# Tani843/Mixed_Precision_Multigrid_Solvers_for_PDEs

Measured on AMD Instinct MI355X. Metric: MDoF/s per V-cycle on 2D Poisson, higher is better.
Workload: dtype f64 (adaptive policy); 1 GPU; 2D Poisson 4097^2 adaptive fp32->fp64 (switch_threshold=1e-6), V(2,2) weighted-Jacobi omega=0.8, 11 levels, 1xMI355X; levels=11, cycle=V(2,2), smoother=jacobi, parallelism=1 GPU

## Files before the change

### include/mghip.h

```cpp
#ifndef MGHIP_H
#define MGHIP_H

#include <stdint.h>

#ifdef __cplusplus
extern "C" {
#endif

#define MG_OK 0
#define MG_ERR_INVALID_VALUE (-1)
#define MG_ERR_NO_DEVICE (-2)
#define MG_ERR_HIP (-3)
#define MG_ERR_STATE (-4)
#define MG_ERR_ALLOC (-5)

typedef enum { MG_F32 = 0, MG_F64 = 1 } mg_dtype;
typedef enum {
  MG_JACOBI = 0,
  MG_RBGS = 1,
  MG_LEXGS = 2
} mg_smoother_t;
typedef enum { MG_CYCLE_V = 0, MG_CYCLE_W = 1, MG_CYCLE_F = 2 } mg_cycle_t;
typedef enum {
  MG_PREC_DOUBLE = 0,
// ... 16 lines not shown
  double coarse_tol;
  int32_t coarse_maxit;
  int32_t precision;
  double switch_threshold;
  double memory_threshold_gb;
  int32_t adaptive_reference_rule;
  int32_t device;
  int32_t profile;
  int32_t colour_offset;
  int32_t fused;
  int32_t tail;
  int32_t fmg_cycles;
  int32_t speculate;
  int32_t coarse_direct;
  int32_t mixed_split;
} mg_config;

typedef struct mg_stats {
  double solve_seconds;
  double h2d_seconds;
  double d2h_seconds;
  double initial_residual;
  int32_t precision_switches;
  int32_t last_coarse_sweeps;
  int32_t switch_reason;
  double fp32_floor;
} mg_stats;

typedef struct mg_handle mg_handle;

// ... 145 lines not shown
```

### mixed_precision_multigrid_solvers_for_pdes_amd/_lib.py

```python
import ctypes as C
import os

import numpy as np

from . import _build

MG_OK = 0
MG_ERR_INVALID_VALUE, MG_ERR_NO_DEVICE, MG_ERR_HIP, MG_ERR_STATE, MG_ERR_ALLOC, MG_ERR_TIMEOUT = -1, -2, -3, -4, -5, -6
MG_PLAN_PHASES = 7
PLAN_PHASE_NAMES = ("legs", "halo_copy", "halo_exchange", "coarse_allgather", "replicated_engine", "allreduce", "other")


class PlanTimeout(RuntimeError):
    """mg_plan_wait gave up (MG_ERR_TIMEOUT): the queued device work is still queued, so the process must not
    synchronise on it again -- report and leave (distributed.bench_main does, with os._exit)."""
MG_F32, MG_F64 = 0, 1
MG_JACOBI, MG_RBGS, MG_LEXGS = 0, 1, 2
MG_CYCLE_V, MG_CYCLE_W, MG_CYCLE_F = 0, 1, 2
MG_PREC_DOUBLE, MG_PREC_SINGLE, MG_PREC_MIXED_LEVELS, MG_PREC_ADAPTIVE, MG_PREC_SINGLE_MANAGED, MG_PREC_DEFECT = 0, 1, 2, 3, 4, 5

CYCLES = {"V": MG_CYCLE_V, "W": MG_CYCLE_W, "F": MG_CYCLE_F}


class MgConfig(C.Structure):
    _fields_ = [
        ("nx", C.c_int32), ("ny", C.c_int32),
        ("x0", C.c_double), ("x1", C.c_double), ("y0", C.c_double), ("y1", C.c_double),
        ("coeff", C.c_double),
        ("max_levels", C.c_int32), ("cycle", C.c_int32), ("pre", C.c_int32), ("post", C.c_int32),
        ("smoother", C.c_int32),
        ("omega", C.c_double),
        ("coarse_tol", C.c_double), ("coarse_maxit", C.c_int32),
        ("precision", C.c_int32),
        ("switch_threshold", C.c_double), ("memory_threshold_gb", C.c_double),
        ("adaptive_reference_rule", C.c_int32),
        ("device", C.c_int32), ("profile", C.c_int32), ("colour_offset", C.c_int32), ("fused", C.c_int32),
        ("tail", C.c_int32), ("fmg_cycles", C.c_int32), ("speculate", C.c_int32), ("coarse_direct", C.c_int32),
        ("mixed_split", C.c_int32),
    ]


class MgStats(C.Structure):
    _fields_ = [
        ("solve_seconds", C.c_double), ("h2d_seconds", C.c_double), ("d2h_seconds", C.c_double),
        ("initial_residual", C.c_double),
        ("precision_switches", C.c_int32), ("last_coarse_sweeps", C.c_int32),
        ("switch_reason", C.c_int32), ("fp32_floor", C.c_double),
    ]


SWITCH_REASONS = {0: None, 1: "threshold", 2: "stagnation", 3: "fp32_floor", 4: "fp32_skipped"}


# ... 195 lines not shown
```

### mixed_precision_multigrid_solvers_for_pdes_amd/csrc/mg_engine.hip

```cpp
#include "mg_launch.hpp"

#include <cstring>

namespace mgh {

std::string& last_error() {
  thread_local std::string msg;
  return msg;
}

static int upload(std::string* err, void* dev, int ddt, int ld, const void* host, int hdt, int nx, int ny, void* staging,
           hipStream_t st) {
  if (ddt == hdt) {
    HIPC(err, hipMemcpy2DAsync(dev, (size_t)ld * esize(ddt), host, (size_t)ny * esize(hdt), (size_t)ny * esize(hdt), nx,
                               hipMemcpyHostToDevice, st));
  } else {
    const int lds = pitch_elems(hdt, ny);
    HIPC(err, hipMemcpy2DAsync(staging, (size_t)lds * esize(hdt), host, (size_t)ny * esize(hdt), (size_t)ny * esize(hdt),
                               nx, hipMemcpyHostToDevice, st));
    d_convert(hdt, ddt, staging, dev, nx, ny, lds, ld, st);
  }
  HIPC(err, hipStreamSynchronize(st));
  return MG_OK;
}
// ... 267 lines not shown
  if ((tail2 || tail_lds) && h->cfg.tail != 0) {
    if (h->tail_direct && h->tail_minv_sigma != h->sigma) { const int rc = build_coarse_inverse(h); if (rc != MG_OK) return rc; }
    if (tail2) return tail2_launch(h, zero_u);
    launch_tail(h, zero_u);
    return MG_OK;
  }
  if (l == L - 1) {
    coarse_solve(h, l, zero_u);
    return MG_OK;
  }
  Level& c = h->lv[l + 1];
  const int dc = h->level_dtype(l + 1);
  const bool fine = (l == 0);
  const int sm = h->cfg.smoother;
  LegGeom g = leg_geom(h, l, dt, dc);
  if (part != kPartBack) {
    StageTimer tm(h, &f, 0);
    if (h->cfg.pre > 2 && zero_u) { (void)hipMemsetAsync(f.u[dt], 0, bytes, h->stream); zero_u = false; }
    extra_sweeps(h, f, dt, g, h->cfg.pre - 2);
    g.nsweep = std::min(2, h->cfg.pre);
    d_down(sm, dt, dc, f.u[dt], f.rhs[dt], f.t[dt], c.rhs[dc], g, zero_u, h->stream);
    std::swap(f.u[dt], f.t[dt]);
  }
  for (int k = 0, n = h->visits(l); k < n && part != kPartBack; ++k) {
    const int rc = cycle_fused(h, l + 1, k == 0);
    if (rc != MG_OK) return rc;
  }
  if (part != kPartFront) {
    StageTimer tm(h, &f, 2);
    const bool want_norm = fine && h->cfg.post <= 2 && h->cfg.precision != MG_PREC_DEFECT;
    g.nsweep = std::min(2, h->cfg.post);
    const int n = d_up(sm, dt, dc, h->grid_dtype, f.u[dt], f.rhs[dt], f.t[dt], c.u[dc], h->partials, g, want_norm, h->stream);
    if (n < 0) return MG_ERR_INVALID_VALUE;
    std::swap(f.u[dt], f.t[dt]);
    if (fine) h->norm_partials = want_norm ? n : 0;
    extra_sweeps(h, f, dt, g, h->cfg.post - 2);
  }
  return MG_OK;
}

bool span_ok(const mg_handle* h) {
  if (h->cfg.speculate < 2 || !h->fused() || h->L() < 3 || h->varcoef) return false;
  if (h->cfg.pre < 1 || h->cfg.pre > 2 || h->cfg.post < 1 || h->cfg.post > 2 || h->cfg.precision == MG_PREC_DEFECT) return false;
  if (!use_rb(leg_geom(h, 0, h->level_dtype(0), h->level_dtype(1)))) return false;
  return h->level_dtype(0) == h->level_dtype(1) && (h->level_dtype(0) == MG_F32 || h->grid_dtype == MG_F64);
}
int cycle_span(mg_handle* h, bool keep_mid) {
// ... 468 lines not shown
    const int rc = run_cycle(h);
    if (rc != MG_OK) return fail(&h->err, rc, "cycle: unsupported precision combination");
  }
  HIPC(&h->err, hipGetLastError());
  return MG_OK;
}

int mg_time_op(mg_handle* h, int op, int level, int dtype, int reps, double* avg_ms) {
  if (!h || !avg_ms || reps < 1 || level < 0 || level >= h->L() || !valid_dtype(dtype))
    return fail(h ? &h->err : nullptr, MG_ERR_INVALID_VALUE, "mg_time_op: bad argument");
  HIPC(&h->err, hipSetDevice(h->cfg.device));
  Level& v = h->lv[level];
  const int dt = dtype;
  if (op != 6 && (!v.u[dt] || !v.rhs[dt])) return fail(&h->err, MG_ERR_STATE, "mg_time_op: level has no arrays of that dtype");
  if ((op == 0 || op == 10) && h->cfg.smoother != MG_JACOBI) return fail(&h->err, MG_ERR_STATE, "mg_time_op: jacobi needs a Jacobi-configured handle");
  if ((op == 0 || (op >= 7 && op <= 9)) && !v.t[dt]) return fail(&h->err, MG_ERR_STATE, "mg_time_op: no ping-pong buffer on this level");
  if ((op == 2 || op == 4 || op == 5 || op == 7 || op == 8) && (level >= h->L() - 1 || !v.r[dt])) return fail(&h->err, MG_ERR_STATE, "mg_time_op: no coarser level");
  static const int exp_nsweep = exp_env("MG_EXP_NSWEEP", 2);
  h->norm_partials = 0;
  if (level == 0 && (op == 0 || op == 1 || (op >= 5 && op <= 9) || op == 12 || op == 13)) h->iterate_zero = false;
  std::vector<void*> hbm_sets;
  struct FreeSets { std::vector<void*>& v; ~FreeSets() { for (void* p : v) (void)hipFree(p); } } free_sets{hbm_sets};
  int nsets = 0, set_idx = 0;
  if (op == 10 || op == 11) {
    const size_t bytes = (size_t)v.nx * v.ld[dt] * esize(dt);
    nsets = std::max<int>(3, (int)((768ull << 20) / (3 * bytes)) + 1);
    for (int k = 0; k < 3 * nsets; ++k) {
      void* p = nullptr;
      HIPC(&h->err, hipMalloc(&p, bytes));
      hbm_sets.push_back(p);
      HIPC(&h->err, hipMemcpyAsync(p, (k % 3 == 1) ? v.rhs[dt] : v.u[dt], bytes, hipMemcpyDeviceToDevice, h->stream));
    }
  }
  hipEvent_t e0, e1;
  HIPC(&h->err, hipEventCreate(&e0));
// ... 22 lines not shown
                  std::swap(v.u[dt], v.t[dt]); } break;
        case 8: { Level& c = h->lv[level + 1]; const int dc = c.u[dt] ? dt : 1 - dt;
                  LegGeom g = leg_geom(h, level, dt, dc); g.nsweep = exp_nsweep;
                  if (d_up(h->cfg.smoother, dt, dc, h->grid_dtype, v.u[dt], v.rhs[dt], v.t[dt], c.u[dc], h->partials, g, level == 0, h->stream) < 0) return MG_ERR_INVALID_VALUE;
                  std::swap(v.u[dt], v.t[dt]); } break;
        case 9: { LegGeom g = leg_geom(h, level, dt, -1); g.nsweep = exp_nsweep;
                  d_sweeps(h->cfg.smoother, dt, v.u[dt], v.rhs[dt], v.t[dt], g, h->stream);
                  std::swap(v.u[dt], v.t[dt]); } break;
        case 12: case 13: {
                  const int phase0 = h->phase;
                  if (h->cfg.precision == MG_PREC_ADAPTIVE) h->phase = dt;
                  const bool ok = level == 0 && span_ok(h) && h->level_dtype(0) == dt;
                  const int rc2 = ok ? cycle_span(h, op == 12) : MG_ERR_INVALID_VALUE;
                  h->phase = phase0;
                  if (rc2 != MG_OK) return rc2; } break;
        default: return MG_ERR_INVALID_VALUE;
      }
    }
    return MG_OK;
  };
  int rc = run(1);
  if (rc != MG_OK) { (void)hipEventDestroy(e0); (void)hipEventDestroy(e1); return fail(&h->err, rc, "mg_time_op: unsupported op"); }
  HIPC(&h->err, hipEventRecord(e0, h->stream));
  rc = run(reps);
  HIPC(&h->err, hipEventRecord(e1, h->stream));
  HIPC(&h->err, hipEventSynchronize(e1));
  float ms = 0;
  HIPC(&h->err, hipEventElapsedTime(&ms, e0, e1));
  (void)hipEventDestroy(e0); (void)hipEventDestroy(e1);
  *avg_ms = (double)ms / reps;
// ... 5 lines not shown
```

### mixed_precision_multigrid_solvers_for_pdes_amd/csrc/mg_kernels.hpp

```cpp
#pragma once

#include <hip/hip_runtime.h>
#include <stdint.h>
#include <type_traits>

namespace mg {

constexpr int kBlock = 256;
constexpr int kTileRowBytes = 512;
constexpr int kTI = 32;
constexpr int kNumXcd = 8;
constexpr int kCoarseTag = 0, kFineTag = 1;
constexpr int kSmJacobi = 0, kSmRbgs = 1;
__host__ __device__ constexpr int sweep_halo(int sm) { return sm == kSmRbgs ? 2 : 1; }

template <typename T> struct VecW { static constexpr int N = 16 / sizeof(T); };

template <typename T> struct alignas(16) Pack {
  T v[VecW<T>::N];
};

template <typename T> __device__ __forceinline__ Pack<T> ldg(const T* p) {
  return *reinterpret_cast<const Pack<T>*>(p);
}
// ... 1546 lines not shown
    }
  }
  Pack<T> f[S::RPT], uu[S::RPT];
#pragma unroll
  for (int k = 0; k < S::RPT; ++k) {
    const int r = r_base + k, gi = ri0 + r;
    f[k] = zero_pack<T>();
    uu[k] = zero_pack<T>();
    if (!worker || r >= S::RI) continue;
    if (gi >= 0 && gi < a.nx && gj0 >= 0 && gj0 < a.nyv && !MG_EXP_NO_LOAD) {
      f[k] = ldg(rhs + (size_t)gi * a.ld + gj0);
      if (!ZERO_INIT) uu[k] = ldg(u + (size_t)gi * a.ld + gj0);
    }
  }
  if (PROLONG) __syncthreads();
#pragma unroll
  for (int k = 0; k < S::RPT; ++k) {
    const int r = r_base + k, gi = ri0 + r;
    if (!worker || r >= S::RI) continue;
    if (PROLONG && gi >= 0 && gi < a.nx && gj0 >= 0 && gj0 < a.nyv && !MG_EXP_NO_LOAD) {
      using TS = typename std::conditional<(sizeof(TC) > sizeof(T)), TC, T>::type;
      TC val[N];
      bool ok[N];
      const TX* pe = patch - ((ptrdiff_t)pic0 * PW + pjc0);
      prolong_vec<TX, TC, N>(pe, PW, a.nxc, a.nyc, gi, gj0, a.nx, a.ny, a.sides, val, ok, a.ci_off, a.cj_off);
#pragma unroll
      for (int e = 0; e < N; ++e)
        if (ok[e]) uu[k].v[e] = (T)((TS)uu[k].v[e] + (TS)val[e]);
    }
    *reinterpret_cast<Pack<T>*>(bufA + r * S::RJ + lc) = uu[k];
  }
  __syncthreads();

  T* src = bufA;
  T* dst = bufB;
  if (SM == kSmRbgs) {
    for (int s = 0; s < 2 * a.nsweep; ++s) {
      const int colour = s & 1;
#pragma unroll
      for (int k = 0; k < S::RPT; ++k) {
        const int r = r_base + k, gi = ri0 + r;
        if (!worker || r >= S::RI) continue;
        if (r >= 1 && r < S::RI - 1 && gi >= 1 && gi < a.nx - 1) {
          const Pack<T> up = *reinterpret_cast<const Pack<T>*>(src + (r - 1) * S::RJ + lc);
          const Pack<T> mid = *reinterpret_cast<const Pack<T>*>(src + r * S::RJ + lc);
          const Pack<T> dn = *reinterpret_cast<const Pack<T>*>(src + (r + 1) * S::RJ + lc);
          const T left = src[r * S::RJ + lc - 1];
          const T right = src[r * S::RJ + lc + N];
          Pack<T> o = mid;
#pragma unroll
          for (int e = 0; e < N; ++e) {
            const T w = (e == 0) ? left : mid.v[e - 1];
// ... 6 lines not shown
              un = (f[k].v[e] + (ihx2 * sx + ihy2 * sy)) * rdv[VAR ? k : 0][VAR ? e : 0];
            } else {
              const T nb = ihx2 * (dn.v[e] + up.v[e]) + ihy2 * (ea + w);
              un = a.use_div ? (f[k].v[e] + nb) / D : (f[k].v[e] + nb) * invD;
            }
            const T res = one_m_omega * mid.v[e] + omega * un;
            const int gj = gj0 + e;
            if (gj >= 1 && gj < a.ny - 1 && (((gi + gj + a.colour_offset) & 1) == colour)) o.v[e] = res;
          }
          *reinterpret_cast<Pack<T>*>(src + r * S::RJ + lc) = o;
        }
      }
      __syncthreads();
    }
  } else
  for (int s = 0; s < (MG_EXP_NO_COMPUTE ? 0 : a.nsweep); ++s) {
    if (worker && r_base < S::RI) {
      Pack<T> up = (r_base >= 1) ? *reinterpret_cast<const Pack<T>*>(src + (r_base - 1) * S::RJ + lc) : zero_pack<T>();
      Pack<T> mid = *reinterpret_cast<const Pack<T>*>(src + r_base * S::RJ + lc);
#pragma unroll
      for (int k = 0; k < S::RPT; ++k) {
        const int r = r_base + k, gi = ri0 + r;
        if (r >= S::RI) break;
        const Pack<T> dn = (r + 1 < S::RI) ? *reinterpret_cast<const Pack<T>*>(src + (r + 1) * S::RJ + lc) : zero_pack<T>();
        Pack<T> o = mid;
        if (r >= 1 && r < S::RI - 1 && gi >= 1 && gi < a.nx - 1) {
          const T left = src[r * S::RJ + lc - 1];
          const T right = src[r * S::RJ + lc + N];
#pragma unroll
          for (int e = 0; e < N; ++e) {
            const T w = (e == 0) ? left : mid.v[e - 1];
// ... 119 lines not shown
```

### mixed_precision_multigrid_solvers_for_pdes_amd/csrc/mg_launch.hip

```cpp
#include "mg_launch.hpp"
#include "mg_rb_kernels.hpp"

#include <cstring>

namespace mgh {

int pitch_elems(int dt, int ny) {
  const size_t bytes = ((size_t)ny * esize(dt) + 511) / 512 * 512;
  return (int)(bytes / esize(dt));
}

template <typename T>
mg::TileGeom make_geom(int nx, int ny, int ld, bool interior_only) {
  using S = mg::TileShape<T>;
  mg::TileGeom g;
  g.nx = nx; g.ny = ny; g.ld = ld;
  g.nyv = std::min(ld, (ny + S::N - 1) / S::N * S::N);
  g.i_org = interior_only ? 1 : 0;
  const int rows = interior_only ? nx - 2 : nx;
  const int cols = interior_only ? ny - 1 : ny;
  const int tiles_i = (rows + mg::kTI - 1) / mg::kTI;
  g.tiles_j = (cols + S::TJ - 1) / S::TJ;
  g.ntiles = tiles_i * g.tiles_j;
  return g;
// ... 332 lines not shown
    using T = decltype(t); using TX = decltype(x); using TC = decltype(tc);
    if constexpr (!interp_ok<T, TX, TC>) return -1;
    else return with_smoother(sm, [&](auto s) {
      constexpr int SM = decltype(s)::value;
      return norm ? launch_leg_sized<kLegUpNorm, T, TX, TC, SM>(u, rhs, out, e_c, partials, g, false, st)
                  : launch_leg_sized<kLegUp, T, TX, TC, SM>(u, rhs, out, e_c, partials, g, false, st);
    });
  });
}
void d_sweeps(int sm, int dt, const void* u, const void* rhs, void* out, const LegGeom& g, hipStream_t st) {
  with_dtype(dt, [&](auto t) {
    using T = decltype(t);
    with_smoother(sm, [&](auto s) {
      launch_leg_sized<kLegSweeps, T, T, T, decltype(s)::value>(u, rhs, out, nullptr, nullptr, g, false, st);
    });
  });
}

void d_inject_ring(int di, int dout, const void* fine, void* coarse, int nxf, int nyf, int ldf, int nxc, int nyc, int ldc,
                   hipStream_t st, int sides, int ci_off, int cj_off) {
  with_dtype(di, dout, [&](auto ti, auto to) {
    using TI = decltype(ti); using TO = decltype(to);
    hipLaunchKernelGGL((mg::inject_ring_kernel<TI, TO>), dim3(grid_for(2 * (nxc + nyc))), dim3(mg::kBlock), 0, st,
                       (const TI*)fine, (TO*)coarse, nxf, nyf, ldf, nxc, nyc, ldc, sides, ci_off, cj_off);
  });
}
void d_var(int mode, int dt, const void* u, const void* a, const void* f, void* out, int nx, int ny, int ld, double hx, double hy,
           double omega, double coeff, int colour, int poff, hipStream_t st, double sigma) {
  auto go = [&](auto m) { launch_var<decltype(m)::value>(dt, u, a, f, out, nullptr, nx, ny, ld, hx, hy, omega, coeff, colour, poff, st, sigma); };
  if (mode == mg::kVarJacobi) go(std::integral_constant<int, mg::kVarJacobi>());
// ... 127 lines not shown
```

### mixed_precision_multigrid_solvers_for_pdes_amd/csrc/mg_launch.hpp

```cpp
#pragma once

#include "mg_host.hpp"

namespace mgh {

int pitch_elems(int dt, int ny);
size_t max_partials(int nx, int ny);

void d_jacobi(int dt, const void* u, const void* rhs, void* out, int nx, int ny, int ld, double hx, double hy,
              double omega, hipStream_t st, bool fine = false, double sigma = 0.0);
void d_rbgs_colour(int dt, void* u, const void* rhs, int nx, int ny, int ld, double hx, double hy, double omega,
                   int colour, int poff, hipStream_t st, bool fine = false, double sigma = 0.0);
void d_residual(int dt, const void* u, const void* f, void* r, int nx, int ny, int ld, double hx, double hy,
                double coeff, hipStream_t st, bool fine = false, double sigma = 0.0);
int d_residual_norm(int dt, const void* u, const void* f, double* partials, int nx, int ny, int ld, double hx,
                    double hy, double coeff, hipStream_t st, bool fine = false, double sigma = 0.0);
int d_sumsq(int dt, const void* x, double* partials, int ld, int i_lo, int i_hi, int j_lo, int j_hi, hipStream_t st);
void launch_reduce(const double* partials, int n, double* out, hipStream_t st, mg::HostMailbox* mailbox = nullptr,
                   unsigned long long seq = 0);
void d_restrict_sub(int di, int dout, const void* fine, void* coarse, int ldf, int nxc, int nyc, int ldc, int sides,
                    hipStream_t st);
void d_restrict(int di, int dout, const void* fine, void* coarse, int nxf, int nyf, int ldf, int ldc, hipStream_t st);
int d_prolong_sub(bool add, int dc, int df, int dcomp, const void* e, void* u, int nxf, int nyf, int ldf, int nxc, int nyc,
                  int ldc, int sides, hipStream_t st);
// ... 23 lines not shown
  int select = 0, in_i_lo = 0, in_i_hi = 0, in_j_lo = 0, in_j_hi = 0;
  double sigma = 0.0;
  const void* acoef = nullptr;
  const void* rdiag = nullptr;
  int rb = 0;
};
bool use_rb(const LegGeom& g);

int d_span(int dt, int dcomp, const void* u, const void* rhs, void* out_mid, void* out_next, const void* e_c, void* rhs_c,
           double* partials, const LegGeom& g, int nsweep_pre, hipStream_t st, int sm = MG_JACOBI);
void d_down(int sm, int dt, int dx, const void* u, const void* rhs, void* out, void* rhs_c, const LegGeom& g, bool zero_init,
            hipStream_t st);
int d_up(int sm, int dt, int dx, int dcomp, const void* u, const void* rhs, void* out, const void* e_c, double* partials,
         const LegGeom& g, bool norm, hipStream_t st);
void d_sweeps(int sm, int dt, const void* u, const void* rhs, void* out, const LegGeom& g, hipStream_t st);

constexpr size_t kTailPoolLimit = 150 * 1024;
size_t tail_pool_bytes(const mg_handle* h, int k, size_t esz, size_t esz_last);
int tail_set_attrs(size_t bytes);
void launch_tail(mg_handle* h, bool zero_top);

int launch_defect(mg_handle* h, bool update);
void d_stream_triad(int dt, const void* a, const void* b, void* out, int nx, int ny, int ld, hipStream_t st);
void d_residual_f32in_f64out(const float* u, const float* f, double* r, int nx, int ny, int ld_in, int ld_out, double hx,
                             double hy, double coeff, hipStream_t st);

}
```

### mixed_precision_multigrid_solvers_for_pdes_amd/csrc/mg_rb_kernels.hpp

```cpp
#pragma once

#include "mg_kernels.hpp"

namespace mg {

#ifndef MG_RB_HL_MIN
#define MG_RB_HL_MIN 4
#endif
template <typename T, int HALO, int W, int RPT> struct RbShape {
  static constexpr int N = VecW<T>::N;
  static constexpr int HL = (MG_RB_HL_MIN <= 2 && 2 * N >= HALO) ? 2 : ((HALO + N - 1) / N > 4 ? (HALO + N - 1) / N : 4);
  static constexpr int RI = W * RPT;
  static constexpr int RJ = 64 * N;
  static constexpr int TI = RI - 2 * HALO;
  static constexpr int TJ = (64 - 2 * HL) * N;
  static_assert(TI > 0 && TI % 2 == 0, "tile height must be even (coarse rows sit on every other tile row)");
  static_assert(RPT % 2 == 0, "rows per wave must be even (row parities are compile-time constants per strip row)");
  static_assert(HL * N >= HALO, "lateral halo too narrow");
};

#ifndef MG_RB_NT_MODE
#define MG_RB_NT_MODE 3
#endif
template <typename T> __device__ __forceinline__ T dpp_from_lower_lane(T x);
// ... 68 lines not shown
    return r;
  }
};

template <typename T, int W>
__device__ __forceinline__ void rb_exchange(Pack<T>* __restrict__ xb, int w, int lane, const Pack<T>& top, const Pack<T>& bottom,
                                            Pack<T>& above, Pack<T>& below) {
  xb[(w * 2 + 0) * 64 + lane] = top;
  xb[(w * 2 + 1) * 64 + lane] = bottom;
  __syncthreads();
  above = (w > 0) ? xb[((w - 1) * 2 + 1) * 64 + lane] : zero_pack<T>();
  below = (w < W - 1) ? xb[((w + 1) * 2 + 0) * 64 + lane] : zero_pack<T>();
}

template <typename T, int HALO, bool PROLONG, int POST, bool ZERO_INIT, typename TX, typename TC, int SM, int W, int RPT, bool INT, int NT,
          bool VAR, int SPAN = 0>
__device__ __forceinline__ void rb_leg_body(const T* __restrict__ u, const T* __restrict__ rhs, T* __restrict__ out,
                                            const TX* __restrict__ e_coarse, TX* __restrict__ rhs_coarse,
                                            double* __restrict__ partials, const FusedArgs& a, T ihx2, T ihy2, T invD, T D, T omega,
                                            T one_m_omega, T coeff, Pack<T>* __restrict__ xbuf, TX* __restrict__ patch,
                                            double* __restrict__ red, int i0, int j0, const T* __restrict__ acoef, T sigma,
                                            const T* __restrict__ rdiag, T* __restrict__ out2 = nullptr) {
  static_assert(SPAN == 0 || (PROLONG && POST == kPostRestrict && !ZERO_INIT), "a spanning leg is an up leg followed by a down leg");
  using S = RbShape<T, HALO, W, RPT>;
  constexpr int N = S::N;
  constexpr int PH = S::RI / 2 + 2, PW = S::RJ / 2 + 2;
  constexpr int kRowPar = (1 - HALO) & 1;
  const int ri0 = i0 - HALO, rj0 = j0 - S::HL * N;
  const int lane = threadIdx.x & 63, w = __builtin_amdgcn_readfirstlane(threadIdx.x >> 6);
  const int gj0 = rj0 + lane * N;
  const int r_base = w * RPT;
  const bool col_in = INT || (gj0 >= 0 && gj0 < a.nyv);

  const int pic0 = (ri0 >> 1) + a.ci_off, pjc0 = (rj0 >> 1) + a.cj_off;
  if (PROLONG) {
    for (int idx = threadIdx.x; idx < PH * PW; idx += W * 64) {
      const int pr = idx / PW, pc = idx - pr * PW;
      const int ic = pic0 + pr, jc = pjc0 + pc;
// ... 32 lines not shown
#pragma unroll
    for (int k = 0; k < RPT; ++k) {
      const Pack<T> up = (k > 0) ? A[k > 0 ? k - 1 : 0] : a_above;
      const Pack<T> dn = (k < RPT - 1) ? A[k < RPT - 1 ? k + 1 : 0] : a_below;
      const T left = dpp_from_lower_lane<T>(A[k].v[N - 1]);
      const T right = dpp_from_upper_lane<T>(A[k].v[0]);
#pragma unroll
      for (int e = 0; e < N; ++e) {
        av[VAR ? k : 0].v[e] = T(0.5) * (A[k].v[e] + up.v[e]);
        if (k == RPT - 1) av[VAR ? RPT : 0].v[e] = T(0.5) * (A[k].v[e] + dn.v[e]);
        ah[VAR ? k : 0][VAR ? e : 0] = T(0.5) * (A[k].v[e] + ((e == 0) ? left : A[k].v[e > 0 ? e - 1 : 0]));
      }
      ah[VAR ? k : 0][VAR ? N : 0] = T(0.5) * (A[k].v[N - 1] + right);
    }
  }
  if (PROLONG) {
    __syncthreads();
    using TS = typename std::conditional<(sizeof(TC) > sizeof(T)), TC, T>::type;
    if (INT) {
      constexpr int M = N / 2 + 1;
      const TX* pl = patch + (r_base / 2) * PW + lane * (N / 2);
#pragma unroll
      for (int k = 0; k < RPT; ++k) {
        const bool iodd = ((kRowPar + k) & 1) != 0;
        const int pr = (k + kRowPar) >> 1;
        TC av[M], bv[M];
#pragma unroll
        for (int m = 0; m < M; ++m) {
          av[m] = (TC)pl[pr * PW + m];
          bv[m] = iodd ? (TC)pl[(pr + 1) * PW + m] : TC(0);
        }
// ... 9 lines not shown
    } else {
      const TX* pe = patch - ((ptrdiff_t)pic0 * PW + pjc0);
#pragma unroll
      for (int k = 0; k < RPT; ++k) {
        const int gi = ri0 + r_base + k;
        if (gi >= 0 && gi < a.nx && col_in) {
          TC val[N];
          bool ok[N];
          prolong_vec<TX, TC, N>(pe, PW, a.nxc, a.nyc, gi, gj0, a.nx, a.ny, a.sides, val, ok, a.ci_off, a.cj_off);
#pragma unroll
          for (int e = 0; e < N; ++e)
            if (ok[e]) U[k].v[e] = (T)((TS)U[k].v[e] + (TS)val[e]);
        }
      }
    }
  }

  int stage = 0;
  auto run_sweeps = [&](int nsw) {
  const int npass = (SM == kSmRbgs) ? 2 * nsw : nsw;
  for (int s = 0; s < npass; ++s, ++stage) {
    Pack<T> above, below;
    rb_exchange<T, W>(xbuf + (size_t)(stage & 1) * W * 2 * 64, w, lane, U[0], U[RPT - 1], above, below);
    const int colour = s & 1;
    static_assert(N % 2 == 0 && RPT % 2 == 0, "strip rows / lane cells must be even for a workgroup-uniform colour parity");
    const int par0 = (ri0 + rj0 + a.colour_offset) & 1;
    auto pass = [&](auto qp) {
      constexpr int QP = decltype(qp)::value;
      Pack<T> prev = above;
#pragma unroll
      for (int k = 0; k < RPT; ++k) {
        const int r = r_base + k, gi = ri0 + r;
        const Pack<T> mid = U[k];
        const Pack<T> dn = (k < RPT - 1) ? U[k + 1] : below;
        const T left = dpp_from_lower_lane<T>(mid.v[N - 1]);
        const T right = dpp_from_upper_lane<T>(mid.v[0]);
// ... 20 lines not shown
            const T sx = aip * dn.v[e] + aim * prev.v[e], sy = ajp * ea + ajm * wv;
            const T un = (F[k].v[e] + (ihx2 * sx + ihy2 * sy)) * RD[VAR ? k : 0].v[e];
            const T res = one_m_omega * mid.v[e] + omega * un;
            const int gj = gj0 + e;
            if (INT || (gj >= 1 && gj < a.ny - 1)) o.v[e] = res;
          }
        }
        U[k] = o;
        prev = (SM == kSmRbgs) ? o : mid;
      }
    };
    if (SM == kSmRbgs && ((par0 + colour) & 1) != 0) pass(std::integral_constant<int, 1>{});
    else pass(std::integral_constant<int, 0>{});
  }
  };
  run_sweeps(a.nsweep);

  const bool lane_in_tile = lane >= S::HL && lane < 64 - S::HL;
  auto store_tile = [&](T* __restrict__ dst) {
#pragma unroll
    for (int k = 0; k < RPT; ++k) {
      const int r = r_base + k, gi = ri0 + r;
      if (r >= HALO && r < HALO + S::TI && lane_in_tile && (INT || (gi < a.nx && gj0 < a.nyv))) {
        if (NT & 1) stg_nt(dst + (size_t)gi * a.ld + gj0, U[k]); else stg(dst + (size_t)gi * a.ld + gj0, U[k]);
      }
    }
  };
  if (SPAN != 2) store_tile(out);
  if (POST == kPostNone) return;

  Pack<T> R[RPT];
  double acc = 0.0;
  auto residual = [&](auto norm_stage) {
    constexpr bool NORM = decltype(norm_stage)::value;
    Pack<T> above, below;
    rb_exchange<T, W>(xbuf + (size_t)(stage & 1) * W * 2 * 64, w, lane, U[0], U[RPT - 1], above, below);
    ++stage;
#pragma unroll
    for (int k = 0; k < RPT; ++k) {
      const int r = r_base + k, gi = ri0 + r;
      const Pack<T> up = (k > 0) ? U[k - 1] : above;
      const Pack<T> mid = U[k];
      const Pack<T> dn = (k < RPT - 1) ? U[k + 1] : below;
// ... 37 lines not shown
            if (NORM && in_tile && (INT || (gi >= a.ni_lo && gi < a.ni_hi && gj >= a.nj_lo && gj < a.nj_hi)))
              acc += (double)o.v[e] * (double)o.v[e];
          }
        }
      }
      R[k] = o;
    }
  };
  if (POST == kPostNorm || SPAN) {
    residual(std::true_type{});
    const double t = block_reduce_sum<W>(acc, red);
    if (threadIdx.x == 0) partials[blockIdx.x] = t;
    if (!SPAN) return;
  }
  if (SPAN) {
    run_sweeps(a.nsweep2);
    store_tile(out2);
  }
  residual(std::false_type{});

  {
    Pack<T> above, below;
    rb_exchange<T, W>(xbuf + (size_t)(stage & 1) * W * 2 * 64, w, lane, R[0], R[RPT - 1], above, below);
#pragma unroll
    for (int k = 0; k < RPT; ++k) {
      const int r = r_base + k, fi = ri0 + r;
      const Pack<T> up = (k > 0) ? R[k - 1] : above;
      const Pack<T> mid = R[k];
      const Pack<T> dn = (k < RPT - 1) ? R[k + 1] : below;
      if (((kRowPar + k) & 1) != 0) continue;
      const T nw0 = dpp_from_lower_lane<T>(up.v[N - 1]), w0 = dpp_from_lower_lane<T>(mid.v[N - 1]), sw0 = dpp_from_lower_lane<T>(dn.v[N - 1]);
// ... 3 lines not shown
#pragma unroll
      for (int e = 0; e < N; e += 2) {
        const int fj = gj0 + e, jc = (fj >> 1) + a.cj_off;
        if (!INT && (jc < 1 || jc > a.nyc - 2 || fj < 1 || fj > a.ny - 2)) continue;
        const T NWv = (e == 0) ? nw0 : up.v[e > 0 ? e - 1 : 0], Wv = (e == 0) ? w0 : mid.v[e > 0 ? e - 1 : 0],
                SWv = (e == 0) ? sw0 : dn.v[e > 0 ? e - 1 : 0];
        const T corners = ((NWv + up.v[e + 1]) + SWv) + dn.v[e + 1];
        const T edges = ((up.v[e] + dn.v[e]) + Wv) + mid.v[e + 1];
        rhs_coarse[(size_t)ic * a.ldc + jc] = (TX)((T(1.0 / 16.0) * corners + T(1.0 / 8.0) * edges) + T(1.0 / 4.0) * mid.v[e]);
      }
    }
  }
}

template <typename T, int HALO, bool PROLONG, int POST, bool ZERO_INIT, typename TX, typename TC, int TAG, int SM, int W, int RPT,
          bool VAR = false>
__global__ __launch_bounds__(W * 64, (VAR && sizeof(T) == 8) ? 4 : 1) void rb_leg_kernel(
    const T* __restrict__ u, const T* __restrict__ rhs, T* __restrict__ out,
    const TX* __restrict__ e_coarse,
    TX* __restrict__ rhs_coarse,
    double* __restrict__ partials,
    FusedArgs a, T ihx2, T ihy2, T invD, T D, T omega, T one_m_omega, T coeff,
    const T* __restrict__ acoef,
    T sigma,
    const T* __restrict__ rdiag) {
  using S = RbShape<T, HALO, W, RPT>;
  constexpr int N = S::N;
  constexpr int kNT = (TAG == 2) ? MG_RB_NT_MODE : 0;
  constexpr int PH = S::RI / 2 + 2, PW = S::RJ / 2 + 2;
  constexpr size_t kXBytes = (size_t)2 * W * 2 * 64 * sizeof(Pack<T>);
  constexpr size_t kPatchBytes = PROLONG ? (size_t)PH * PW * sizeof(TX) : 0;
// ... 12 lines not shown
    if ((a.select == 1) != inner) {
      if (POST == kPostNorm && threadIdx.x == 0) partials[blockIdx.x] = 0.0;
      return;
    }
  }
  bool interior = !(a.exp_flags & 4) && ri0 >= 1 && ri0 + S::RI <= a.nx - 1 && rj0 >= 1 && rj0 + S::RJ <= a.ny - 1;
  if (PROLONG) {
    const int pic0 = (ri0 >> 1) + a.ci_off, pjc0 = (rj0 >> 1) + a.cj_off;
    interior = interior && pic0 >= 0 && pic0 + PH <= a.nxc && pjc0 >= 0 && pjc0 + PW <= a.nyc;
  }
  if (POST == kPostNorm) interior = interior && i0 >= a.ni_lo && i0 + S::TI <= a.ni_hi && j0 >= a.nj_lo && j0 + S::TJ <= a.nj_hi;
  if (POST == kPostRestrict)
    interior = interior && ((i0 + 1) >> 1) + a.ci_off >= 1 && ((i0 + S::TI - 1) >> 1) + a.ci_off <= a.nxc - 2 &&
               (j0 >> 1) + a.cj_off >= 1 && ((j0 + S::TJ - 2) >> 1) + a.cj_off <= a.nyc - 2;
  if (interior)
    rb_leg_body<T, HALO, PROLONG, POST, ZERO_INIT, TX, TC, SM, W, RPT, true, kNT, VAR>(u, rhs, out, e_coarse, rhs_coarse, partials, a, ihx2, ihy2,
                                                                                invD, D, omega, one_m_omega, coeff, xbuf, patch, red, i0, j0,
                                                                                acoef, sigma, rdiag);
  else
    rb_leg_body<T, HALO, PROLONG, POST, ZERO_INIT, TX, TC, SM, W, RPT, false, kNT, VAR>(u, rhs, out, e_coarse, rhs_coarse, partials, a, ihx2, ihy2,
                                                                                 invD, D, omega, one_m_omega, coeff, xbuf, patch, red, i0, j0,
                                                                                 acoef, sigma, rdiag);
}

template <typename T, int HALO, typename TX, typename TC, int TAG, int SM, int W, int RPT, int SPAN>
__global__ __launch_bounds__(W * 64, 4) void rb_span_kernel(
    const T* __restrict__ u, const T* __restrict__ rhs, T* __restrict__ out_mid, T* __restrict__ out_next,
    const TX* __restrict__ e_coarse, TX* __restrict__ rhs_coarse, double* __restrict__ partials,
    FusedArgs a, T ihx2, T ihy2, T invD, T D, T omega, T one_m_omega, T coeff) {
  using S = RbShape<T, HALO, W, RPT>;
  constexpr int N = S::N;
  constexpr int kNT = (TAG == 2) ? MG_RB_NT_MODE : 0;
  constexpr int PH = S::RI / 2 + 2, PW = S::RJ / 2 + 2;
  constexpr size_t kXBytes = (size_t)2 * W * 2 * 64 * sizeof(Pack<T>);
  constexpr size_t kPatchBytes = (size_t)PH * PW * sizeof(TX);
// ... 33 lines not shown
```

### mixed_precision_multigrid_solvers_for_pdes_amd/engine.py

```python
import ctypes as C

import numpy as np

from . import _lib


def _direct_code(coarse_direct):
    import os
    if coarse_direct is None:
        coarse_direct = {"0": False, "1": True}.get(os.environ.get("MG_COARSE_DIRECT", "auto"), "auto")
    if isinstance(coarse_direct, str):
        if coarse_direct != "auto":
            raise ValueError(f"coarse_direct: True, False, 'auto' or None, not {coarse_direct!r}")
        return -1
    return int(bool(coarse_direct))


class MultigridEngine:

    def __init__(self, nx, ny, domain=(0.0, 1.0, 0.0, 1.0), coeff=-1.0, max_levels=4, cycle="V", pre=2, post=2,
                 smoother=_lib.MG_JACOBI, omega=0.8, coarse_tol=1e-12, coarse_maxit=1000,
                 precision=_lib.MG_PREC_DOUBLE, switch_threshold=1e-6, memory_threshold_gb=4.0,
                 adaptive_reference_rule=False, device=0, profile=False, colour_offset=0, fused=2, tail=True, speculate=True, fmg_cycles=0,
                 mixed_split=0, coarse_direct=None):
        lib = _lib.load()
        if isinstance(cycle, str):
            if cycle not in _lib.CYCLES:
                raise ValueError(f"unknown cycle type {cycle!r}")
            cycle = _lib.CYCLES[cycle]
        cfg = _lib.MgConfig(int(nx), int(ny), float(domain[0]), float(domain[1]), float(domain[2]), float(domain[3]),
                            float(coeff), int(max_levels), int(cycle), int(pre), int(post), int(smoother),
                            float(omega), float(coarse_tol), int(coarse_maxit), int(precision),
                            float(switch_threshold), float(memory_threshold_gb), int(bool(adaptive_reference_rule)),
                            int(device), int(bool(profile)), int(colour_offset), int(fused), int(tail), int(fmg_cycles), (2 if speculate is True else int(speculate)),
                            _direct_code(coarse_direct), int(mixed_split))
        self.cfg = cfg
        self._h = C.c_void_p(None)
        _lib.check(lib.mg_create(C.byref(cfg), C.byref(self._h)))
        self._lib = lib
        n = C.c_int(0)
        self._check(lib.mg_num_levels(self._h, C.byref(n)))
        self.num_levels = n.value
        self.shapes = []
        for l in range(self.num_levels):
            a, b = C.c_int(0), C.c_int(0)
            self._check(lib.mg_level_shape(self._h, l, C.byref(a), C.byref(b)))
            self.shapes.append((a.value, b.value))
        self.nx, self.ny = int(nx), int(ny)

    def _check(self, rc):
# ... 95 lines not shown
        self._check(self._lib.mg_fmg(self._h, int(cycles_per_level)))

    def residual_norm(self):
        out = C.c_double(0.0)
        self._check(self._lib.mg_residual_norm(self._h, C.byref(out)))
        return out.value

    def set_working_precision(self, dtype):
        self._check(self._lib.mg_set_working_precision(self._h, _lib.dtype_code(dtype)))

    def synchronize(self):
        self._check(self._lib.mg_synchronize(self._h))

    def time_op(self, op, level=0, dtype=np.float64, reps=20):
        ops = {"jacobi": 0, "rbgs": 1, "residual": 2, "residual_norm": 3, "restrict": 4, "prolong": 5, "cycle": 6,
               "down_leg": 7, "up_leg": 8, "sweeps2": 9, "jacobi_hbm": 10, "stream_hbm": 11, "span_leg": 12, "span_leg_nomid": 13}
        out = C.c_double(0.0)
        self._check(self._lib.mg_time_op(self._h, ops[op] if isinstance(op, str) else int(op), int(level),
                                         _lib.dtype_code(dtype), int(reps), C.byref(out)))
        return out.value

    def level_timings(self):
        res = {}
        for l in range(self.num_levels):
            t = (C.c_double * 3)()
            self._check(self._lib.mg_level_timings(self._h, l, t))
            res[l] = {"smooth_time": t[0], "restrict_time": t[1], "prolong_time": t[2]}
        return res
```

Before: 79320 MDoF/s.

## Recompute zero-start pre-smoothed iterate in up leg instead of storing it

On coarse levels where the iterate starts at zero, the down leg no longer writes the pre-smoothed solution. The up leg regenerates it from the rhs before adding the prolonged correction and post-smoothing. The first Jacobi sweep from a zero start is also replaced by a closed form (omega*rhs/D), which skips the neighbour exchange. This cuts HBM write and read traffic for the iterate at the cost of redoing the pre-smoothing sweeps in the up leg. A new config flag, on by default, gates the path, and timing ops are added for it.

```diff
diff --git a/include/mghip.h b/include/mghip.h
--- a/include/mghip.h
+++ b/include/mghip.h
@@ -54,6 +54,7 @@
   int32_t speculate;
   int32_t coarse_direct;
   int32_t mixed_split;
+  int32_t recompute;
 } mg_config;
 
 typedef struct mg_stats {
diff --git a/mixed_precision_multigrid_solvers_for_pdes_amd/_lib.py b/mixed_precision_multigrid_solvers_for_pdes_amd/_lib.py
--- a/mixed_precision_multigrid_solvers_for_pdes_amd/_lib.py
+++ b/mixed_precision_multigrid_solvers_for_pdes_amd/_lib.py
@@ -36,7 +36,7 @@
         ("adaptive_reference_rule", C.c_int32),
         ("device", C.c_int32), ("profile", C.c_int32), ("colour_offset", C.c_int32), ("fused", C.c_int32),
         ("tail", C.c_int32), ("fmg_cycles", C.c_int32), ("speculate", C.c_int32), ("coarse_direct", C.c_int32),
-        ("mixed_split", C.c_int32),
+        ("mixed_split", C.c_int32), ("recompute", C.c_int32),
     ]
 
 
diff --git a/mixed_precision_multigrid_solvers_for_pdes_amd/csrc/mg_engine.hip b/mixed_precision_multigrid_solvers_for_pdes_amd/csrc/mg_engine.hip
--- a/mixed_precision_multigrid_solvers_for_pdes_amd/csrc/mg_engine.hip
+++ b/mixed_precision_multigrid_solvers_for_pdes_amd/csrc/mg_engine.hip
@@ -305,13 +305,19 @@
   const bool fine = (l == 0);
   const int sm = h->cfg.smoother;
   LegGeom g = leg_geom(h, l, dt, dc);
+  const bool recompute = zero_u && l >= 1 && part == kPartFull && h->cfg.recompute != 0 && sm == MG_JACOBI && !h->varcoef &&
+                         h->cfg.pre >= 1 && h->cfg.pre <= 2 && recompute_ok(g);
   if (part != kPartBack) {
     StageTimer tm(h, &f, 0);
     if (h->cfg.pre > 2 && zero_u) { (void)hipMemsetAsync(f.u[dt], 0, bytes, h->stream); zero_u = false; }
     extra_sweeps(h, f, dt, g, h->cfg.pre - 2);
     g.nsweep = std::min(2, h->cfg.pre);
-    d_down(sm, dt, dc, f.u[dt], f.rhs[dt], f.t[dt], c.rhs[dc], g, zero_u, h->stream);
-    std::swap(f.u[dt], f.t[dt]);
+    if (recompute) {
+      d_down_nostore(dt, dc, f.rhs[dt], c.rhs[dc], g, h->stream);
+    } else {
+      d_down(sm, dt, dc, f.u[dt], f.rhs[dt], f.t[dt], c.rhs[dc], g, zero_u, h->stream);
+      std::swap(f.u[dt], f.t[dt]);
+    }
   }
   for (int k = 0, n = h->visits(l); k < n && part != kPartBack; ++k) {
     const int rc = cycle_fused(h, l + 1, k == 0);
@@ -321,7 +327,8 @@
     StageTimer tm(h, &f, 2);
     const bool want_norm = fine && h->cfg.post <= 2 && h->cfg.precision != MG_PREC_DEFECT;
     g.nsweep = std::min(2, h->cfg.post);
-    const int n = d_up(sm, dt, dc, h->grid_dtype, f.u[dt], f.rhs[dt], f.t[dt], c.u[dc], h->partials, g, want_norm, h->stream);
+    const int n = recompute ? d_up_recompute(dt, dc, h->grid_dtype, f.rhs[dt], f.t[dt], c.u[dc], g, h->cfg.pre, h->stream)
+                            : d_up(sm, dt, dc, h->grid_dtype, f.u[dt], f.rhs[dt], f.t[dt], c.u[dc], h->partials, g, want_norm, h->stream);
     if (n < 0) return MG_ERR_INVALID_VALUE;
     std::swap(f.u[dt], f.t[dt]);
     if (fine) h->norm_partials = want_norm ? n : 0;
@@ -820,11 +827,11 @@
   const int dt = dtype;
   if (op != 6 && (!v.u[dt] || !v.rhs[dt])) return fail(&h->err, MG_ERR_STATE, "mg_time_op: level has no arrays of that dtype");
   if ((op == 0 || op == 10) && h->cfg.smoother != MG_JACOBI) return fail(&h->err, MG_ERR_STATE, "mg_time_op: jacobi needs a Jacobi-configured handle");
-  if ((op == 0 || (op >= 7 && op <= 9)) && !v.t[dt]) return fail(&h->err, MG_ERR_STATE, "mg_time_op: no ping-pong buffer on this level");
-  if ((op == 2 || op == 4 || op == 5 || op == 7 || op == 8) && (level >= h->L() - 1 || !v.r[dt])) return fail(&h->err, MG_ERR_STATE, "mg_time_op: no coarser level");
+  if ((op == 0 || (op >= 7 && op <= 9) || op == 14 || op == 16) && !v.t[dt]) return fail(&h->err, MG_ERR_STATE, "mg_time_op: no ping-pong buffer on this level");
+  if ((op == 2 || op == 4 || op == 5 || op == 7 || op == 8 || (op >= 14 && op <= 16)) && (level >= h->L() - 1 || !v.r[dt])) return fail(&h->err, MG_ERR_STATE, "mg_time_op: no coarser level");
   static const int exp_nsweep = exp_env("MG_EXP_NSWEEP", 2);
   h->norm_partials = 0;
-  if (level == 0 && (op == 0 || op == 1 || (op >= 5 && op <= 9) || op == 12 || op == 13)) h->iterate_zero = false;
+  if (level == 0 && (op == 0 || op == 1 || (op >= 5 && op <= 9) || (op >= 12 && op <= 16))) h->iterate_zero = false;
   std::vector<void*> hbm_sets;
   struct FreeSets { std::vector<void*>& v; ~FreeSets() { for (void* p : v) (void)hipFree(p); } } free_sets{hbm_sets};
   int nsets = 0, set_idx = 0;
@@ -877,6 +884,18 @@
                   const int rc2 = ok ? cycle_span(h, op == 12) : MG_ERR_INVALID_VALUE;
                   h->phase = phase0;
                   if (rc2 != MG_OK) return rc2; } break;
+        case 14: case 15: case 16: {
+                  Level& c = h->lv[level + 1]; const int dc = (op == 16 ? c.u[dt] : c.rhs[dt]) ? dt : 1 - dt;
+                  LegGeom g = leg_geom(h, level, dt, dc); g.nsweep = exp_nsweep;
+                  if (op == 14) {
+                    d_down(h->cfg.smoother, dt, dc, v.u[dt], v.rhs[dt], v.t[dt], c.rhs[dc], g, true, h->stream);
+                    std::swap(v.u[dt], v.t[dt]);
+                    break;
+                  }
+                  if (h->cfg.smoother != MG_JACOBI || h->varcoef || !recompute_ok(g)) return MG_ERR_INVALID_VALUE;
+                  if (op == 15) { d_down_nostore(dt, dc, v.rhs[dt], c.rhs[dc], g, h->stream); break; }
+                  if (d_up_recompute(dt, dc, h->grid_dtype, v.rhs[dt], v.t[dt], c.u[dc], g, exp_nsweep, h->stream) < 0) return MG_ERR_INVALID_VALUE;
+                  std::swap(v.u[dt], v.t[dt]); } break;
         default: return MG_ERR_INVALID_VALUE;
       }
     }
diff --git a/mixed_precision_multigrid_solvers_for_pdes_amd/csrc/mg_kernels.hpp b/mixed_precision_multigrid_solvers_for_pdes_amd/csrc/mg_kernels.hpp
--- a/mixed_precision_multigrid_solvers_for_pdes_amd/csrc/mg_kernels.hpp
+++ b/mixed_precision_multigrid_solvers_for_pdes_amd/csrc/mg_kernels.hpp
@@ -1584,10 +1584,22 @@
     }
   }
   if (PROLONG) __syncthreads();
+  const int first_pass = (ZERO_INIT && !PROLONG && !VAR && a.nsweep >= 1 && !MG_EXP_NO_COMPUTE) ? 1 : 0;
+  const T zero_nb = ihx2 * T(0) + ihy2 * T(0);
 #pragma unroll
   for (int k = 0; k < S::RPT; ++k) {
     const int r = r_base + k, gi = ri0 + r;
     if (!worker || r >= S::RI) continue;
+    if (first_pass && gi >= 1 && gi < a.nx - 1) {
+#pragma unroll
+      for (int e = 0; e < N; ++e) {
+        const T t = f[k].v[e] + zero_nb;
+        const T un = a.use_div ? t / D : t * invD;
+        const T res = one_m_omega * T(0) + omega * un;
+        const int gj = gj0 + e;
+        if (gj >= 1 && gj < a.ny - 1 && (SM != kSmRbgs || ((gi + gj + a.colour_offset) & 1) == 0)) uu[k].v[e] = res;
+      }
+    }
     if (PROLONG && gi >= 0 && gi < a.nx && gj0 >= 0 && gj0 < a.nyv && !MG_EXP_NO_LOAD) {
       using TS = typename std::conditional<(sizeof(TC) > sizeof(T)), TC, T>::type;
       TC val[N];
@@ -1605,7 +1617,7 @@
   T* src = bufA;
   T* dst = bufB;
   if (SM == kSmRbgs) {
-    for (int s = 0; s < 2 * a.nsweep; ++s) {
+    for (int s = first_pass; s < 2 * a.nsweep; ++s) {
       const int colour = s & 1;
 #pragma unroll
       for (int k = 0; k < S::RPT; ++k) {
@@ -1642,7 +1654,7 @@
       __syncthreads();
     }
   } else
-  for (int s = 0; s < (MG_EXP_NO_COMPUTE ? 0 : a.nsweep); ++s) {
+  for (int s = first_pass; s < (MG_EXP_NO_COMPUTE ? 0 : a.nsweep); ++s) {
     if (worker && r_base < S::RI) {
       Pack<T> up = (r_base >= 1) ? *reinterpret_cast<const Pack<T>*>(src + (r_base - 1) * S::RJ + lc) : zero_pack<T>();
       Pack<T> mid = *reinterpret_cast<const Pack<T>*>(src + r_base * S::RJ + lc);
diff --git a/mixed_precision_multigrid_solvers_for_pdes_amd/csrc/mg_launch.hip b/mixed_precision_multigrid_solvers_for_pdes_amd/csrc/mg_launch.hip
--- a/mixed_precision_multigrid_solvers_for_pdes_amd/csrc/mg_launch.hip
+++ b/mixed_precision_multigrid_solvers_for_pdes_amd/csrc/mg_launch.hip
@@ -370,6 +370,38 @@
     with_smoother(sm, [&](auto s) {
       launch_leg_sized<kLegSweeps, T, T, T, decltype(s)::value>(u, rhs, out, nullptr, nullptr, g, false, st);
     });
+  });
+}
+
+bool recompute_ok(const LegGeom& g) { return use_rb(g) && !g.acoef; }
+
+template <bool UP, typename T, typename TX, typename TC>
+static void launch_recompute(const void* rhs, void* out, const void* coarse, const LegGeom& g, int nsweep_pre, hipStream_t st) {
+  constexpr int SM = mg::kSmJacobi, W = MG_EXP_RB_W, RPT = 8;
+  constexpr int HALO = 2 * mg::sweep_halo(SM) + (UP ? 1 : 2);
+  constexpr int POST = UP ? mg::kPostNone : mg::kPostRestrict;
+  const Coef c = coefs(g.hx, g.hy, g.sigma);
+  mg::FusedArgs a = rb_args<T, HALO, W, RPT>(g, !c.pow2);
+  a.nsweep2 = nsweep_pre;
+  auto k = rb_stream(g, sizeof(T)) ? mg::rb_leg_kernel<T, HALO, UP, POST, true, TX, TC, 2, SM, W, RPT, false, UP>
+                                   : mg::rb_leg_kernel<T, HALO, UP, POST, true, TX, TC, 1, SM, W, RPT, false, UP>;
+  hipLaunchKernelGGL(k, dim3(a.ntiles), dim3(W * 64), 0, st, (const T*)nullptr, (const T*)rhs, (T*)out,
+                     UP ? (const TX*)coarse : nullptr, UP ? nullptr : (TX*)coarse, (double*)nullptr, a, (T)c.ihx2, (T)c.ihy2,
+                     (T)c.invD, (T)c.diag, (T)g.omega, (T)(1.0 - g.omega), (T)(UP ? 0.0 : g.coeff), (const T*)nullptr, (T)g.sigma,
+                     (const T*)nullptr);
+}
+void d_down_nostore(int dt, int dx, const void* rhs, void* rhs_c, const LegGeom& g, hipStream_t st) {
+  with_dtype(dt, dx, [&](auto t, auto x) {
+    using T = decltype(t);
+    launch_recompute<false, T, decltype(x), T>(rhs, nullptr, rhs_c, g, 0, st);
+  });
+}
+int d_up_recompute(int dt, int dx, int dcomp, const void* rhs, void* out, const void* e_c, const LegGeom& g, int nsweep_pre,
+                   hipStream_t st) {
+  return with_dtype(dt, dx, dcomp, [&](auto t, auto x, auto tc) {
+    using T = decltype(t); using TX = decltype(x); using TC = decltype(tc);
+    if constexpr (!interp_ok<T, TX, TC>) return -1;
+    else { launch_recompute<true, T, TX, TC>(rhs, out, e_c, g, nsweep_pre, st); return 0; }
   });
 }
 
diff --git a/mixed_precision_multigrid_solvers_for_pdes_amd/csrc/mg_launch.hpp b/mixed_precision_multigrid_solvers_for_pdes_amd/csrc/mg_launch.hpp
--- a/mixed_precision_multigrid_solvers_for_pdes_amd/csrc/mg_launch.hpp
+++ b/mixed_precision_multigrid_solvers_for_pdes_amd/csrc/mg_launch.hpp
@@ -61,6 +61,10 @@
 int d_up(int sm, int dt, int dx, int dcomp, const void* u, const void* rhs, void* out, const void* e_c, double* partials,
          const LegGeom& g, bool norm, hipStream_t st);
 void d_sweeps(int sm, int dt, const void* u, const void* rhs, void* out, const LegGeom& g, hipStream_t st);
+bool recompute_ok(const LegGeom& g);
+void d_down_nostore(int dt, int dx, const void* rhs, void* rhs_c, const LegGeom& g, hipStream_t st);
+int d_up_recompute(int dt, int dx, int dcomp, const void* rhs, void* out, const void* e_c, const LegGeom& g, int nsweep_pre,
+                   hipStream_t st);
 
 constexpr size_t kTailPoolLimit = 150 * 1024;
 size_t tail_pool_bytes(const mg_handle* h, int k, size_t esz, size_t esz_last);
diff --git a/mixed_precision_multigrid_solvers_for_pdes_amd/csrc/mg_rb_kernels.hpp b/mixed_precision_multigrid_solvers_for_pdes_amd/csrc/mg_rb_kernels.hpp
--- a/mixed_precision_multigrid_solvers_for_pdes_amd/csrc/mg_rb_kernels.hpp
+++ b/mixed_precision_multigrid_solvers_for_pdes_amd/csrc/mg_rb_kernels.hpp
@@ -106,7 +106,7 @@
 }
 
 template <typename T, int HALO, bool PROLONG, int POST, bool ZERO_INIT, typename TX, typename TC, int SM, int W, int RPT, bool INT, int NT,
-          bool VAR, int SPAN = 0>
+          bool VAR, int SPAN = 0, bool STORE = true>
 __device__ __forceinline__ void rb_leg_body(const T* __restrict__ u, const T* __restrict__ rhs, T* __restrict__ out,
                                             const TX* __restrict__ e_coarse, TX* __restrict__ rhs_coarse,
                                             double* __restrict__ partials, const FusedArgs& a, T ihx2, T ihy2, T invD, T D, T omega,
@@ -114,6 +114,8 @@
                                             double* __restrict__ red, int i0, int j0, const T* __restrict__ acoef, T sigma,
                                             const T* __restrict__ rdiag, T* __restrict__ out2 = nullptr) {
   static_assert(SPAN == 0 || (PROLONG && POST == kPostRestrict && !ZERO_INIT), "a spanning leg is an up leg followed by a down leg");
+  static_assert(STORE || (ZERO_INIT && !PROLONG && POST == kPostRestrict && SPAN == 0), "only the zero-start down leg may drop its iterate");
+  static_assert(!(ZERO_INIT && PROLONG) || (SM == kSmJacobi && !VAR && POST == kPostNone), "the recomputing up leg: Jacobi, constant coefficients");
   using S = RbShape<T, HALO, W, RPT>;
   constexpr int N = S::N;
   constexpr int PH = S::RI / 2 + 2, PW = S::RJ / 2 + 2;
@@ -176,7 +178,8 @@
       ah[VAR ? k : 0][VAR ? N : 0] = T(0.5) * (A[k].v[N - 1] + right);
     }
   }
-  if (PROLONG) {
+  auto prolong_add = [&]() {
+    if (!PROLONG) return;
     __syncthreads();
     using TS = typename std::conditional<(sizeof(TC) > sizeof(T)), TC, T>::type;
     if (INT) {
@@ -216,12 +219,36 @@
         }
       }
     }
-  }
+  };
 
   int stage = 0;
-  auto run_sweeps = [&](int nsw) {
+  auto zero_pass = [&](auto qp) {
+    constexpr int QP = decltype(qp)::value;
+    const T z = ihx2 * T(0) + ihy2 * T(0);
+#pragma unroll
+    for (int k = 0; k < RPT; ++k) {
+      const int gi = ri0 + r_base + k;
+      if (!INT && !(gi >= 1 && gi < a.nx - 1)) continue;
+#pragma unroll
+      for (int e = 0; e < N; ++e) {
+        const T t = F[k].v[e] + z;
+        const T un = (a.use_div != 0) ? t / D : t * invD;
+        const T res = one_m_omega * T(0) + omega * un;
+        const int gj = gj0 + e;
+        const bool mine = (SM != kSmRbgs) || (((QP + k + e) & 1) == 0);
+        if ((INT || (gj >= 1 && gj < a.ny - 1)) && mine) U[k].v[e] = res;
+      }
+    }
+  };
+  auto run_sweeps = [&](int nsw, bool from_zero) {
   const int npass = (SM == kSmRbgs) ? 2 * nsw : nsw;
-  for (int s = 0; s < npass; ++s, ++stage) {
+  int s = 0;
+  if (ZERO_INIT && !VAR && from_zero && npass > 0) {
+    if (SM == kSmRbgs && ((ri0 + rj0 + a.colour_offset) & 1) != 0) zero_pass(std::integral_constant<int, 1>{});
+    else zero_pass(std::integral_constant<int, 0>{});
+    s = 1;
+  }
+  for (; s < npass; ++s, ++stage) {
     Pack<T> above, below;
     rb_exchange<T, W>(xbuf + (size_t)(stage & 1) * W * 2 * 64, w, lane, U[0], U[RPT - 1], above, below);
     const int colour = s & 1;
@@ -272,7 +299,14 @@
     else pass(std::integral_constant<int, 0>{});
   }
   };
-  run_sweeps(a.nsweep);
+  if (ZERO_INIT && PROLONG) {
+    run_sweeps(a.nsweep2, true);
+    prolong_add();
+    run_sweeps(a.nsweep, false);
+  } else {
+    prolong_add();
+    run_sweeps(a.nsweep, ZERO_INIT);
+  }
 
   const bool lane_in_tile = lane >= S::HL && lane < 64 - S::HL;
   auto store_tile = [&](T* __restrict__ dst) {
@@ -284,7 +318,7 @@
       }
     }
   };
-  if (SPAN != 2) store_tile(out);
+  if (SPAN != 2 && STORE) store_tile(out);
   if (POST == kPostNone) return;
 
   Pack<T> R[RPT];
@@ -352,7 +386,7 @@
     if (!SPAN) return;
   }
   if (SPAN) {
-    run_sweeps(a.nsweep2);
+    run_sweeps(a.nsweep2, false);
     store_tile(out2);
   }
   residual(std::false_type{});
@@ -386,7 +420,7 @@
 }
 
 template <typename T, int HALO, bool PROLONG, int POST, bool ZERO_INIT, typename TX, typename TC, int TAG, int SM, int W, int RPT,
-          bool VAR = false>
+          bool VAR = false, bool STORE = true>
 __global__ __launch_bounds__(W * 64, (VAR && sizeof(T) == 8) ? 4 : 1) void rb_leg_kernel(
     const T* __restrict__ u, const T* __restrict__ rhs, T* __restrict__ out,
     const TX* __restrict__ e_coarse,
@@ -429,11 +463,11 @@
     interior = interior && ((i0 + 1) >> 1) + a.ci_off >= 1 && ((i0 + S::TI - 1) >> 1) + a.ci_off <= a.nxc - 2 &&
                (j0 >> 1) + a.cj_off >= 1 && ((j0 + S::TJ - 2) >> 1) + a.cj_off <= a.nyc - 2;
   if (interior)
-    rb_leg_body<T, HALO, PROLONG, POST, ZERO_INIT, TX, TC, SM, W, RPT, true, kNT, VAR>(u, rhs, out, e_coarse, rhs_coarse, partials, a, ihx2, ihy2,
+    rb_leg_body<T, HALO, PROLONG, POST, ZERO_INIT, TX, TC, SM, W, RPT, true, kNT, VAR, 0, STORE>(u, rhs, out, e_coarse, rhs_coarse, partials, a, ihx2, ihy2,
                                                                                 invD, D, omega, one_m_omega, coeff, xbuf, patch, red, i0, j0,
                                                                                 acoef, sigma, rdiag);
   else
-    rb_leg_body<T, HALO, PROLONG, POST, ZERO_INIT, TX, TC, SM, W, RPT, false, kNT, VAR>(u, rhs, out, e_coarse, rhs_coarse, partials, a, ihx2, ihy2,
+    rb_leg_body<T, HALO, PROLONG, POST, ZERO_INIT, TX, TC, SM, W, RPT, false, kNT, VAR, 0, STORE>(u, rhs, out, e_coarse, rhs_coarse, partials, a, ihx2, ihy2,
                                                                                  invD, D, omega, one_m_omega, coeff, xbuf, patch, red, i0, j0,
                                                                                  acoef, sigma, rdiag);
 }
diff --git a/mixed_precision_multigrid_solvers_for_pdes_amd/engine.py b/mixed_precision_multigrid_solvers_for_pdes_amd/engine.py
--- a/mixed_precision_multigrid_solvers_for_pdes_amd/engine.py
+++ b/mixed_precision_multigrid_solvers_for_pdes_amd/engine.py
@@ -22,7 +22,7 @@
                  smoother=_lib.MG_JACOBI, omega=0.8, coarse_tol=1e-12, coarse_maxit=1000,
                  precision=_lib.MG_PREC_DOUBLE, switch_threshold=1e-6, memory_threshold_gb=4.0,
                  adaptive_reference_rule=False, device=0, profile=False, colour_offset=0, fused=2, tail=True, speculate=True, fmg_cycles=0,
-                 mixed_split=0, coarse_direct=None):
+                 mixed_split=0, coarse_direct=None, recompute=True):
         lib = _lib.load()
         if isinstance(cycle, str):
             if cycle not in _lib.CYCLES:
@@ -33,7 +33,7 @@
                             float(omega), float(coarse_tol), int(coarse_maxit), int(precision),
                             float(switch_threshold), float(memory_threshold_gb), int(bool(adaptive_reference_rule)),
                             int(device), int(bool(profile)), int(colour_offset), int(fused), int(tail), int(fmg_cycles), (2 if speculate is True else int(speculate)),
-                            _direct_code(coarse_direct), int(mixed_split))
+                            _direct_code(coarse_direct), int(mixed_split), int(bool(recompute)))
         self.cfg = cfg
         self._h = C.c_void_p(None)
         _lib.check(lib.mg_create(C.byref(cfg), C.byref(self._h)))
@@ -159,7 +159,8 @@
 
     def time_op(self, op, level=0, dtype=np.float64, reps=20):
         ops = {"jacobi": 0, "rbgs": 1, "residual": 2, "residual_norm": 3, "restrict": 4, "prolong": 5, "cycle": 6,
-               "down_leg": 7, "up_leg": 8, "sweeps2": 9, "jacobi_hbm": 10, "stream_hbm": 11, "span_leg": 12, "span_leg_nomid": 13}
+               "down_leg": 7, "up_leg": 8, "sweeps2": 9, "jacobi_hbm": 10, "stream_hbm": 11, "span_leg": 12, "span_leg_nomid": 13,
+               "down_leg_zero": 14, "down_leg_zero_nostore": 15, "up_leg_recompute": 16}
         out = C.c_double(0.0)
         self._check(self._lib.mg_time_op(self._h, ops[op] if isinstance(op, str) else int(op), int(level),
                                          _lib.dtype_code(dtype), int(reps), C.byref(out)))
```

Result: no change. 78690 MDoF/s (-0.8%).
